# fegennari/3DWorld

Measured on AMD Instinct MI355X. Metric: heightmap Gcells/sec (noise+erosion), 16384^2 grid, higher is better.
Workload: dtype f32

## Files before the change

### 3dworld_amd/csrc/terra_driver.hpp

```cpp
#pragma once
#include "terra_common.hpp"
#include "terra_noise.hpp"
#include "terra_erosion.hpp"
#include "terra_landscape.hpp"
#include "terra_modmap.hpp"
#include "terra_treemap.hpp"
#include "terra_treeplace.hpp"
#include "terra_decidplace.hpp"
#include "terra_sceneryplace.hpp"
#include "terra_treeao.hpp"
#include "terra_treeedit.hpp"
#include "../../include/terra.h"
#include <vector>
#include <map>
#include <string>
#include <algorithm>
#include <cmath>
#include <stdexcept>
#include <string.h>
#include <stdio.h>
#include <stdlib.h>

namespace terra {

// ... 306 lines not shown
	for (int dy = -1; dy <= 1; ++dy) {
		for (int dx = -1; dx <= 1; ++dx) {
			if (dx == 0 && dy == 0) continue;
			float z0 = z_start;
			int stepx = dx, stepy = dy, vx = x, vy = y;
			for (unsigned s = 0; s < 8; ++s) {
				vx += stepx; vy += stepy;
				z0 += dz;
				stepx += dx; stepy += dy;
				if (ctx(vx + 36, vy + 36) > z0) {atten += (8 - s); break;}
			}
		}
	}
	float const ao_scale = (float)(1.0 - (double)((float)atten/(float)64));
	return (uint8_t)(255.0*(double)ao_scale);
}

TERRA_HD float rsq_approx(float x) {
#if defined(__HIP_DEVICE_COMPILE__)
	return __builtin_amdgcn_rsqf(x);
#else
	return (float)(1.0/sqrt((double)x));
#endif
}
TERRA_HD void tile_normal_v(float zc, float zr, float zd, float dxv, float dyv, float dxy, float nv[3]) {
	nv[0] = dyv*(zc - zr); nv[1] = dxv*(zc - zd); nv[2] = dxy;
	float const mag = sqrtf(nv[0]*nv[0] + nv[1]*nv[1] + nv[2]*nv[2]);
	if (!(mag < 1.0E-12f)) {nv[0] /= mag; nv[1] /= mag; nv[2] /= mag;}
}
TERRA_HD void tile_normal_zv(float const *z, unsigned zv, unsigned x, unsigned y, float dxv, float dyv, float dxy, float nv[3]) {
	unsigned const ix2 = y*zv + x;
	tile_normal_v(z[ix2], z[ix2 + 1], z[ix2 + zv], dxv, dyv, dxy, nv);
}

struct options_t {
	int gen_fused = 0;
	int ero_lead = 2;
	int ero_batch = 0;
	int ero_fuse = 3;
	int ero_sparse = -1;
	int ero_sparse_retraces = -1;
	int ero_live = 1;
	int ero_diag = 0;
	int ero_ck_steps = 0, ero_ck_max = -1;
	bool ero_near_set = false; int ero_near = 0;
	long long ero_mem_budget = -1;
	int simple_kernels = 0;
	int ao_bands = 1;
	int ao_whole = 1;
	int voxels_cols = 1;
	int graphs = 1;
	int sg_kc = 27, sg_kc_tiles = 27;
	int sg_rowgroup = 4;
	int tile_erosion_window = 0;
	int weights_simple = 0;
	int shadows_levels = 0;
	bool set(char const *key, char const *value) {
		if (!key || !value) return false;
		std::string const k(key), v(value);
		char *end = nullptr;
		long long const n = strtoll(value, &end, 10);
		bool const is_int = (end != value && *end == '\0');
		auto const flag = [&](int &dst) {if (!is_int || (n != 0 && n != 1)) return false; dst = (int)n; return true;};
		if (k == "gen.fused") {if (!is_int || n < 0 || n > 2) return false; gen_fused = (int)n; return true;}
		if (k == "ero.lead") {if (!is_int || n < 0 || n > 2) return false; ero_lead = (int)n; return true;}
		if (k == "ero.fuse") {if (!is_int || n < 0 || n > 7) return false; ero_fuse = (int)n; return true;}
		if (k == "ero.batch") {if (!is_int || n < 0 || n > (1 << 20)) return false; ero_batch = (int)n; return true;}
		if (k == "ero.sparse") {if (v == "auto") {ero_sparse = -1; return true;} return flag(ero_sparse);}
		if (k == "ero.sparse_retraces") {if (!is_int || n < -1 || n > (1 << 20)) return false; ero_sparse_retraces = (int)n; return true;}
		if (k == "ero.live") return flag(ero_live);
		if (k == "ero.diag") return flag(ero_diag);
		if (k == "ero.ck") {int a = 0, b = 0; if (v == "default") {ero_ck_steps = 0; ero_ck_max = -1; return true;} if (sscanf(value, "%d:%d", &a, &b) != 2 || a < 1 || b < 0 || b > (int)SPEC_CK_MAX) return false; ero_ck_steps = a; ero_ck_max = b; return true;}
		if (k == "ero.near") {if (v == "default") {ero_near_set = false; return true;} if (!is_int || n < -(1 << 20) || n > (1 << 20)) return false; ero_near_set = true; ero_near = (int)n; return true;}
		if (k == "ero.mem_budget") {if (!is_int || n < -1) return false; ero_mem_budget = n; return true;}
		if (k == "kernels.simple") return flag(simple_kernels);
		if (k == "voxels.cols") return flag(voxels_cols);
		if (k == "ao.bands") return flag(ao_bands);
		if (k == "ao.whole") return flag(ao_whole);
		if (k == "graphs") return flag(graphs);
		if (k == "sg.kc") {if (!is_int || (n != 20 && n != 27 && n != 45)) return false; sg_kc = (int)n; return true;}
		if (k == "sg.kc_tiles") {if (!is_int || (n != 27 && n != 45)) return false; sg_kc_tiles = (int)n; return true;}
		if (k == "sg.rowgroup") {if (!is_int || n < 1 || n > 1024) return false; sg_rowgroup = (int)n; return true;}
		if (k == "tile_erosion") {if (v == "lds") {tile_erosion_window = 0; return true;} if (v == "window") {tile_erosion_window = 1; return true;} return false;}
		if (k == "weights.simple") return flag(weights_simple);
		if (k == "shadows.levels") return flag(shadows_levels);
		return false;
	}
};

struct vox_noise_job_t {float l0, l1, l2, v0, v1, v2, o0, o1, o2, frx, fry, mag, freq, zscale; int32_t nn, normalize; uint32_t nx, nz, y0;};
TERRA_HD float voxel_noise_cell(size_t i, vox_noise_job_t const &J, bool perlin) {
	unsigned const z = (unsigned)(i % J.nz), x = (unsigned)((i / J.nz) % J.nx), y = (unsigned)(i / ((size_t)J.nz*J.nx)) + J.y0;
	float const px = ((float)x*J.v0 + J.l0) + J.o0, py = ((float)y*J.v1 + J.l1) + J.o1, pz = ((float)z*J.v2 + J.l2) + J.o2;
	float val = 0.0f, nmag = J.mag, nfreq = (float)(0.25*(double)J.freq);
	for (int n = 0; n < J.nn; ++n) {
		float const ax = nfreq*px + J.frx, ay = nfreq*py + J.fry, az = nfreq*pz + (J.frx - J.fry);
		val += nmag*(perlin ? perlin3(ax, ay, az) : simplex3(ax, ay, az));
		nmag *= 0.5f; nfreq *= 1.92f;
	}
	val += (float)z*J.zscale;
	if (J.normalize) {val = clip_pm1(val);}
	return val;
}

template<bool PERLIN> TERRA_HD nv2 voxel_noise_pair(unsigned x, unsigned y, unsigned z, vox_noise_job_t const &J, char const *tab) {
	float const px = ((float)x*J.v0 + J.l0) + J.o0, py = ((float)y*J.v1 + J.l1) + J.o1;
	nv2 const zf = {(float)z, (float)(z + 1)};
	nv2 const pz = (zf*J.v2 + J.l2) + J.o2;
	nv2 val = {0.0f, 0.0f};
	float nmag = J.mag, nfreq = (float)(0.25*(double)J.freq);
	float const frz = J.frx - J.fry;
	for (int n = 0; n < J.nn; ++n) {
		float const ax = nfreq*px + J.frx, ay = nfreq*py + J.fry;
		nv2 const az = nfreq*pz + frz;
		nv2 const v = PERLIN ? perlin3_lut_z2<true>(ax, ay, az, tab) : simplex3_lut<true>(nv2{ax, ax}, nv2{ay, ay}, az, tab);
		val += nmag*v;
		nmag *= 0.5f; nfreq *= 1.92f;
	}
	val += zf*J.zscale;
	if (J.normalize) {val = nv2{clip_pm1(val[0]), clip_pm1(val[1])};}
	return val;
}

template<class BE> struct terra_engine {
	BE be;
	options_t opt;
	terra_engine() {be.opt = &opt;}
	void set_option(char const *key, char const *value) {
		options_t o = opt;
		if (!o.set(key, value)) throw std::invalid_argument(std::string("terra_set_option: unknown key or bad value: ") + (key ? key : "(null)") + " = " + (value ? value : "(null)"));
		be.sync();
		opt = o;
		be.options_changed();
	}
	terra_config cfg{};
// ... 281 lines not shown
			sk.xconst[k] = ms2*sinTable[k][4] + sinTable[k][2] + x_mult*mx0;
			sk.yconst[k] = ms2*sinTable[k][3] + sinTable[k][1] + y_mult*my0;
			sk.xmdx[k] = x_mult*dx; sk.ymdy[k] = y_mult*dy;
		}
		return sk;
	}

	bool sine_plain_only(int shp, int kstart) const {
		if (shp != 0 || hp.crack_lo < hp.crack_hi || (hp.volcano_width > 0.0f && hp.volcano_height > 0.0f) || consts().custom_glaciate_exp != 0.0f) return false;
		double bound = 0.0;
		for (int k = kstart; k < F_TABLE_SIZE; ++k) {bound += std::fabs((double)(mesh_scale_z_inv*sinTable[k][0]));}
		return (double)min_std(hp.plat_bot, hp.crat_h) > bound*1.001 + 1e-3;
	}

	void gen_grid_dev(float x0, float y0, float dx, float dy, uint32_t nx, uint32_t ny, uint32_t flags, int min_start_sin, float *d_out, float *h_minmax = nullptr, uint32_t row0 = 0, uint32_t nrows = 0xFFFFFFFFu, float *d_minmax = nullptr) {
		require_scene();
		if (nx == 0 || ny == 0) throw std::invalid_argument("build_arrays: nx, ny must be > 0");
		if (nrows == 0xFFFFFFFFu) {if (row0 != 0) throw std::invalid_argument("gen_grid rows: row0 without a row count"); nrows = ny;}
		if (nrows == 0 || row0 >= ny || nrows > ny - row0) throw std::invalid_argument("gen_grid rows: [row0, row0 + nrows) must be a non-empty range inside the grid");
		grid_job_t job;
		job.mx0 = dx*x0; job.my0 = dy*y0; job.mdx = dx; job.mdy = dy; job.nx = nx; job.ny = nrows; job.row0 = row0; ny = nrows;
		job.nxp = round_up(nx, 128); job.nyp = round_up(ny, 128);
		bool const force_sine = (flags & TERRA_GEN_FORCE_SINE) != 0;
		job.mode = force_sine ? (int)MGEN_SINE : mode; job.shape = force_sine ? 0 : shape;
		job.kstart = imax(start_eval_sin, min_start_sin);
		job.glaciate = (flags & TERRA_GEN_GLACIATE) ? 1 : 0;
		job.use_sine_mag = (job.glaciate && hp.sine_mag > 0.0f) ? 1 : 0;
		job.sine_offset = hp.sine_bias*mesh_scale_z_inv;
		job.plain_only = (job.mode == MGEN_SINE && sine_plain_only(job.shape, job.kstart)) ? 1 : 0;
		job.fused = (((flags & (TERRA_GEN_FUSED | TERRA_GEN_FAST)) || opt.gen_fused) && fused_kernel_exists(job.mode, job.plain_only != 0)) ? (((flags & TERRA_GEN_FAST) || opt.gen_fused == 2) ? 2 : 1) : 0;
		job.fast_amax = sine_amp_max(job.kstart);
		noise_consts_t const nc = consts();
		sin_lut_t const L = lut();
		float *smx = scratch<float>(s_smx, job.nxp), *smy = scratch<float>(s_smy, job.nyp);
		uint32_t *d_mm = nullptr;
		bool const sine = (job.mode == MGEN_SINE);
		if (h_minmax || d_minmax || sine) {d_mm = scratch<uint32_t>(s_mm, 2); if (!sine) {be.fill32(d_mm, 0xFFFFFFFFu, 2);}}
		bool fused;
		bool const sm_on = job.use_sine_mag != 0;
		float const sm_scale = hp.sine_mag*mesh_scale_z_inv, sm_freq = mesh_scale*hp.sine_freq, dxi = DX_VAL_INV, dyi = DY_VAL_INV;
		if (sm_on && job.mode != MGEN_SINE) {
			float const mx0 = job.mx0, my0 = job.my0, mdx = dx, mdy = dy;
			uint32_t const nxp = job.nxp, nyp = job.nyp;
			be.launch((size_t)nxp + nyp, [=] TERRA_LAMBDA (size_t i) {
				if (i < nxp) {smx[i] = (i < nx) ? sm_scale*L.COSF(((float)(unsigned)i*mdx + mx0)*dxi*sm_freq) : 0.0f;}
				else {unsigned const y = (unsigned)(i - nxp); smy[y] = (y < ny) ? L.COSF(((float)(y + row0)*mdy + my0)*dyi*sm_freq) : 0.0f;}
			});
		}
		if (job.mode == MGEN_SINE) {
			float const *st = sinTable_dev();
			float const msx = mesh_scale*DX_VAL_INV, msy = mesh_scale*DY_VAL_INV, ms2 = (float)(0.5*(double)mesh_scale), mszi = mesh_scale_z_inv, jmx0 = job.mx0, jmy0 = job.my0, mdx = dx, mdy = dy;
			float *xt = scratch<float>(s_xt, (size_t)F_TABLE_SIZE*job.nxp), *yt = scratch<float>(s_yt, (size_t)F_TABLE_SIZE*job.nyp);
			uint32_t const nxp = job.nxp, nyp = job.nyp;
			size_t const ntab = (size_t)F_TABLE_SIZE*(nxp + nyp);
			uint32_t *const mmz = d_mm;
			be.launch(ntab + (sm_on ? (size_t)nxp + nyp : 0), [=] TERRA_LAMBDA (size_t i) {
				if (i == 0) {mmz[0] = 0xFFFFFFFFu; mmz[1] = 0xFFFFFFFFu;}
				if (i < (size_t)F_TABLE_SIZE*nxp) {
					unsigned const k = (unsigned)(i / nxp), x = (unsigned)(i % nxp);
					float const *stk = st + 5*k;
					float const x_mult = msx*stk[4], xconst = ms2*stk[4] + stk[2] + x_mult*jmx0, xmdx = x_mult*mdx;
					xt[i] = (x < nx) ? L.SINF(xmdx*(float)x + xconst) : 0.0f;
				}
				else if (i < ntab) {
					size_t const j = i - (size_t)F_TABLE_SIZE*nxp;
					unsigned const k = (unsigned)(j / nyp), y = (unsigned)(j % nyp);
					float const *stk = st + 5*k;
					float const y_mult = msy*stk[3], yscale = mszi*stk[0], yconst = ms2*stk[3] + stk[1] + y_mult*jmy0, ymdy = y_mult*mdy;
					yt[j] = (y < ny) ? yscale*L.SINF(ymdy*(float)(y + row0) + yconst) : 0.0f;
				}
				else {
					size_t const q = i - ntab;
					if (q < nxp) {smx[q] = (q < nx) ? sm_scale*L.COSF(((float)(unsigned)q*mdx + jmx0)*dxi*sm_freq) : 0.0f;}
					else {unsigned const y = (unsigned)(q - nxp); smy[y] = (y < ny) ? L.COSF(((float)(y + row0)*mdy + jmy0)*dyi*sm_freq) : 0.0f;}
				}
			});
			fused = be.sine_grid(job, nc, L, xt, yt, smx, smy, d_out, (h_minmax || d_minmax) ? d_mm : nullptr);
		}
		else {fused = be.noise_grid(job, nc, L, smx, smy, d_out, (h_minmax || d_minmax) ? d_mm : nullptr, d_noise_lut);}
		if ((h_minmax || d_minmax) && !fused) {be.minmax(d_out, (size_t)nx*ny, d_mm);}
		if (d_minmax) {uint32_t const *mm = d_mm; be.launch(1, [=] TERRA_LAMBDA (size_t) {d_minmax[0] = ord2f(mm[0]); d_minmax[1] = ord2f(~mm[1]);}, 64);}
		if (h_minmax) {
			uint32_t out[2];
			be.d2h(out, d_mm, sizeof(out));
			h_minmax[0] = ord2f(out[0]); h_minmax[1] = ord2f(~out[1]);
		}
	}

	float eval_mesh_sin_terms(float xv, float yv) const {
		require_scene();
		sin_lut_t const HL = host_lut();
		float zval = 0.0f;
		for (int k = start_eval_sin; k < F_TABLE_SIZE; ++k) {
			float const *stk = sinTable[k];
			zval += stk[0]*HL.SINF(stk[3]*yv + stk[1])*HL.SINF(stk[4]*xv + stk[2]);
		}
		return zval;
	}
	void eval_points_dev(float const *d_xy, uint32_t n, uint32_t kind, float xy_scale, int no_xyoff, int xoff2, int yoff2, float *d_out) {
		require_scene();
		if (n == 0) return;
		if (kind > 1) throw std::invalid_argument("eval_points: kind must be TERRA_POINTS_SCALED or TERRA_POINTS_EXACT");
		noise_consts_t const nc = consts();
		sin_lut_t const L = lut();
		float const *st = sinTable_dev();
		hmap_view_t const hv = hmap_view();
		bool const hm = using_hmap(), hm_detail = using_hmap_with_detail();
		int const md = mode, shp = shape, k0 = start_eval_sin;
		float const half_x = (float)(cfg.mesh_x >> 1), half_y = (float)(cfg.mesh_y >> 1), xss = cfg.scene_x, yss = cfg.scene_y, dxi = DX_VAL_INV, dyi = DY_VAL_INV, msc = mesh_scale, mszi = mesh_scale_z_inv;
		be.launch(n, [=] TERRA_LAMBDA (size_t i) {
			auto const scaled = [&](float xval, float yval, float xys) -> float {
				float const xv = xys*(xval - half_x), yv = xys*(yval - half_y);
				if (md != MGEN_SINE) {
					switch (md) {
					case MGEN_PERLIN:      return noise_zval<MGEN_PERLIN>(xv, yv, shp, nc);
					case MGEN_DWARP_GPU:   return noise_zval<MGEN_DWARP_GPU>(xv, yv, shp, nc);
					case MGEN_SIMPLEX_GPU: return noise_zval<MGEN_SIMPLEX_GPU>(xv, yv, shp, nc);
					default:               return noise_zval<MGEN_SIMPLEX>(xv, yv, shp, nc);
					}
				}
				float const ax = msc*xv, ay = msc*yv;
				float zval = 0.0f;
				for (int k = k0; k < F_TABLE_SIZE; ++k) {float const *stk = st + 5*k; zval += stk[0]*L.SINF(stk[3]*ay + stk[1])*L.SINF(stk[4]*ax + stk[2]);}
				return apply_noise_shape_final(zval*mszi, shp, nc.hp);
// ... 1832 lines not shown
```

### 3dworld_amd/csrc/terra_hip.hip

```cpp
#include "terra_kernels.hpp"
#include "terra_fused.hpp"
#include "terra_fz_api.hpp"
#include "terra_simple_paths.hpp"
#include "terra_xfer.hpp"
#include <stdlib.h>

#define TERRA_HIP_CHECK(expr) do {hipError_t const e_ = (expr); if (e_ != hipSuccess) {throw std::runtime_error(std::string(#expr) + ": " + hipGetErrorString(e_));}} while (0)

struct hip_backend_t : terra::simple_paths<hip_backend_t> {
	int device = -1;
	hipStream_t stream = nullptr, own_stream = nullptr;
	hipEvent_t ev0 = nullptr, ev1 = nullptr;
	terra::options_t const *opt = nullptr;
	bool simple_kernels = false;
	int num_cus = 256;
	float *tile_pad = nullptr; size_t tile_pad_bytes = 0;
	uint32_t *tile_order = nullptr; size_t tile_order_bytes = 0;
	float *vox_p = nullptr; size_t vox_p_bytes = 0;
	bool vox_cols = true;
	int sg_kc = 27;
	unsigned sg_rowgroup = 4;

	static int device_count() {int n = 0; if (hipGetDeviceCount(&n) != hipSuccess) return 0; return n;}
	void init(int dev) {
		device = dev;
		TERRA_HIP_CHECK(hipSetDevice(dev));
		TERRA_HIP_CHECK(hipStreamCreateWithFlags(&own_stream, hipStreamNonBlocking));
		stream = own_stream;
		TERRA_HIP_CHECK(hipEventCreate(&ev0)); TERRA_HIP_CHECK(hipEventCreate(&ev1));
		{int n = 0; if (hipDeviceGetAttribute(&n, hipDeviceAttributeMultiprocessorCount, dev) == hipSuccess && n > 0) {num_cus = n;} else {(void)hipGetLastError();}}
		options_changed();
		TERRA_HIP_CHECK(hipFuncSetAttribute((void const *)terra::k_tile_erosion, hipFuncAttributeMaxDynamicSharedMemorySize, 96*1024));
		TERRA_HIP_CHECK(hipFuncSetAttribute((void const *)terra::k_tile_shadows_level, hipFuncAttributeMaxDynamicSharedMemorySize, 96*1024));
		TERRA_HIP_CHECK(hipFuncSetAttribute((void const *)terra::k_tile_shadows_flow, hipFuncAttributeMaxDynamicSharedMemorySize, 96*1024));
		TERRA_HIP_CHECK(hipFuncSetAttribute((void const *)terra::k_tile_ao<true>, hipFuncAttributeMaxDynamicSharedMemorySize, 64*1024));
		TERRA_HIP_CHECK(hipFuncSetAttribute((void const *)terra::k_tile_ao<false>, hipFuncAttributeMaxDynamicSharedMemorySize, 64*1024));
		ao_tile_ok = hipFuncSetAttribute((void const *)terra::k_tile_ao_tile<true>, hipFuncAttributeMaxDynamicSharedMemorySize, (int)terra::AOT_LDS) == hipSuccess
			&& hipFuncSetAttribute((void const *)terra::k_tile_ao_tile<false>, hipFuncAttributeMaxDynamicSharedMemorySize, (int)terra::AOT_LDS) == hipSuccess;
		if (!ao_tile_ok) {(void)hipGetLastError();}
	}
	void options_changed() {
		if (!opt) return;
		simple_kernels = opt->simple_kernels != 0; sg_kc = opt->sg_kc; sg_rowgroup = (unsigned)opt->sg_rowgroup; vox_cols = opt->voxels_cols != 0;
		if (graphs_enabled != (opt->graphs != 0)) {for (graph_slot_t &g : graphs) {graph_drop(g);} graphs_enabled = opt->graphs != 0;}
	}
	~hip_backend_t() {
		if (pin) (void)hipHostFree(pin);
		if (h3_tab) (void)hipFree(h3_tab);
		if (tile_pad) (void)hipFree(tile_pad);
		if (tile_order) (void)hipFree(tile_order);
		if (tile_acc) (void)hipFree(tile_acc);
		if (tile_map) (void)hipFree(tile_map);
		if (vox_p) (void)hipFree(vox_p);
		if (ev0) (void)hipEventDestroy(ev0);
		if (ev1) (void)hipEventDestroy(ev1);
		for (graph_slot_t &g : graphs) {graph_drop(g);}
		if (relay_ev) (void)hipEventDestroy(relay_ev);
		if (side_stream) (void)hipStreamDestroy(side_stream);
		if (own_stream) (void)hipStreamDestroy(own_stream);
	}
	size_t mem_free() {use(); size_t f = 0, t = 0; if (hipMemGetInfo(&f, &t) != hipSuccess) {(void)hipGetLastError(); return ~(size_t)0 >> 1;} return f;}
	void release_scratch() {
		for (void **p : {(void **)&tile_pad, (void **)&tile_order, (void **)&tile_acc, (void **)&tile_map, (void **)&vox_p}) {if (*p) {(void)hipFree(*p); *p = nullptr;}}
		tile_pad_bytes = tile_order_bytes = tile_acc_bytes = vox_p_bytes = 0; tile_map_count = 0;
	}
	void use() {TERRA_HIP_CHECK(hipSetDevice(device));}
	void set_stream(void *s) {sync(); pin_off = 0; stream = s ? (hipStream_t)s : own_stream;}
	void sync() {use(); TERRA_HIP_CHECK(hipStreamSynchronize(stream));}
	void *alloc(size_t bytes) {use(); void *p = nullptr; TERRA_HIP_CHECK(hipMalloc(&p, bytes ? bytes : 1)); return p;}
	void free(void *p) {use(); (void)hipFree(p);}
	void fill8(void *p, uint8_t v, size_t count) {use(); if (count) TERRA_HIP_CHECK(hipMemsetAsync(p, v, count, stream));}
	void fill32(void *p, uint32_t v, size_t count) {use(); if (count) TERRA_HIP_CHECK(hipMemsetD32Async((hipDeviceptr_t)p, (int)v, count, stream));}
	void h2d(void *d, void const *h, size_t bytes) {
		use();
		if (bytes >= BIG_XFER) {xfer.submit(device, stream, const_cast<void *>(h), d, bytes, true, [this](hipEvent_t e) {return record_via_side(e);}); xfer.wait_all(); return;}
		TERRA_HIP_CHECK(hipMemcpyAsync(d, h, bytes, hipMemcpyHostToDevice, stream)); TERRA_HIP_CHECK(hipStreamSynchronize(stream));
	}
	uint8_t *pin = nullptr; size_t pin_bytes = 0, pin_off = 0; bool pin_failed = false;
	void h2d_async(void *d, void const *h, size_t bytes) {
		if (bytes == 0) return;
		use();
		if (!pin && !pin_failed) {pin_bytes = (size_t)8 << 20; if (hipHostMalloc((void **)&pin, pin_bytes, hipHostMallocDefault) != hipSuccess) {pin = nullptr; pin_bytes = 0; pin_failed = true; (void)hipGetLastError();}}
		size_t const need = (bytes + 255) & ~(size_t)255;
		if (!pin || need > pin_bytes/2) {h2d(d, h, bytes); return;}
		if (pin_off + need > pin_bytes) {TERRA_HIP_CHECK(hipStreamSynchronize(stream)); pin_off = 0;}
		memcpy(pin + pin_off, h, bytes);
		TERRA_HIP_CHECK(hipMemcpyAsync(d, pin + pin_off, bytes, hipMemcpyHostToDevice, stream));
		pin_off += need;
	}
	void d2h(void *h, void const *d, size_t bytes) {
		use();
		if (bytes >= BIG_XFER) {download_async(d, h, bytes); download_wait(); return;}
		TERRA_HIP_CHECK(hipMemcpyAsync(h, d, bytes, hipMemcpyDeviceToHost, stream)); TERRA_HIP_CHECK(hipStreamSynchronize(stream));
	}
	static constexpr size_t BIG_XFER = (size_t)16 << 20;
	terra::xfer_engine_t xfer;
// ... 120 lines not shown

	template<class F> void launch_waves_lean(size_t n, F f) {
		if (n == 0) return;
		use();
		if (n > 0x7FFFFFFFull) throw std::invalid_argument("launch_waves: grid too large");
		hipLaunchKernelGGL(terra::k_waves_lean<F>, dim3((unsigned)n), dim3(64), 0, stream, f);
		TERRA_HIP_CHECK(hipGetLastError());
	}

	template<class F> void launch_waves_nolds(size_t n, F f) {
		if (n == 0) return;
		use();
		if (n > 0x7FFFFFFFull) throw std::invalid_argument("launch_waves: grid too large");
		hipLaunchKernelGGL(terra::k_waves_nolds<F>, dim3((unsigned)n), dim3(64), 0, stream, f);
		TERRA_HIP_CHECK(hipGetLastError());
	}

	void *h3_tab = nullptr; size_t h3_tab_bytes = 0;
	static float h3_scale(float amax) {int e = 0; if (amax > 0.0f && amax < 3.0e38f) {(void)frexpf(amax, &e);} return ldexpf(1.0f, 14 - e);}
	template<int KIND> bool sine_grid_h3(terra::sgf_job_t J, float amax_x, float amax_y, float const *vox_tab = nullptr, uint32_t vnx = 0, uint32_t vny = 0) {
		int const nk = (J.kstart < J.kend) ? J.kend - J.kstart : 0;
		uint32_t const nchunks = (uint32_t)((3*nk + 15)/16);
		if ((uint64_t)std::max(J.nxp, J.nyp)*32u*(nchunks + 1) >= 0xFFFFFFFFull) return false;
		size_t const bx = (size_t)nchunks*J.nxp*32u, by = (size_t)nchunks*J.nyp*32u;
		if (bx + by + 64 > h3_tab_bytes) {if (h3_tab) {sync(); (void)hipFree(h3_tab);} TERRA_HIP_CHECK(hipMalloc(&h3_tab, bx + by + 64)); h3_tab_bytes = bx + by + 64;}
		float const sx = h3_scale(amax_x), sy = h3_scale(amax_y);
		J.xh = h3_tab; J.yh = (char *)h3_tab + bx; J.nchunks = nchunks; J.unscale = 1.0f/(sx*sy);
		if (nchunks && vox_tab) {
			hipLaunchKernelGGL((terra::k_split_voxel_table<false, terra::VOX_SINES>), dim3((J.nxp + 255)/256), dim3(256), 0, stream, vox_tab, vnx, vny, J.nx, J.nxp, sx, (terra::sgh_u4 *)J.xh);
			hipLaunchKernelGGL((terra::k_split_voxel_table<true, terra::VOX_SINES>),  dim3((J.nyp + 255)/256), dim3(256), 0, stream, vox_tab, vnx, vny, J.nx, J.nyp, sy, (terra::sgh_u4 *)J.yh);
		}
		else if (nchunks) {
			hipLaunchKernelGGL(terra::k_split_table<false>, dim3((unsigned)(((size_t)nchunks*J.nxp + 255)/256)), dim3(256), 0, stream, J.xt, J.nxp, J.kstart, J.kend, nchunks, sx, (terra::sgh_u4 *)J.xh);
			hipLaunchKernelGGL(terra::k_split_table<true>,  dim3((unsigned)(((size_t)nchunks*J.nyp + 255)/256)), dim3(256), 0, stream, J.yt, J.nyp, J.kstart, J.kend, nchunks, sy, (terra::sgh_u4 *)J.yh);
		}
		if (KIND == terra::SGF_VOXELS && J.nx <= 64 && (J.nyp % 256u) == 0) {J.narrow = 1; J.ntx = 1; J.nty = J.nyp/256u;}
		unsigned const nb = J.ntx*J.nty, grid = ((nb + 7)/8)*8;
		hipLaunchKernelGGL(terra::k_sine_grid_h3<KIND>, dim3(grid), dim3(256), 0, stream, J);
		TERRA_HIP_CHECK(hipGetLastError());
		return true;
	}
	bool sine_grid(terra::grid_job_t const &job, terra::noise_consts_t const &nc, terra::sin_lut_t const &L, float const *xt, float const *yt, float const *smx, float const *smy, float *out, uint32_t *mm) {
		if (simple_kernels) {sine_grid_simple(job, nc, L, xt, yt, smx, smy, out); return false;}
		use();
		unsigned const ntx = job.nxp/terra::SG_BX, nty = (job.ny + terra::SG_BY - 1)/terra::SG_BY;
		unsigned const nb = ntx*nty, grid = ((nb + 7)/8)*8;
		if (job.fused) {
			terra::sgf_job_t J; memset(&J, 0, sizeof(J));
			J.xt = xt; J.yt = yt; J.smx = smx; J.smy = smy; J.out = out; J.mm = mm; J.nx = job.nx; J.ny = job.ny; J.nxp = job.nxp; J.nyp = job.nyp; J.ntx = ntx; J.nty = nty; J.rowgroup = sg_rowgroup;
			J.kstart = job.kstart; J.kend = terra::F_TABLE_SIZE; J.glaciate = (job.glaciate && nc.glaciate) ? 1 : 0; J.sine_mag = (job.glaciate && job.use_sine_mag) ? 1 : 0;
			J.zmax_est = nc.zmax_est; J.zmax_est2 = nc.zmax_est2; J.zmax_est2_inv = nc.zmax_est2_inv; J.sine_offset = job.sine_offset;
			if (job.fused == 2 && sine_grid_h3<terra::SGF_GRID>(J, 1.0f, job.fast_amax)) return true;
			hipLaunchKernelGGL(terra::k_sine_grid_mx<terra::SGF_GRID>, dim3(std::min(grid, (unsigned)(2*num_cus + 7)/8*8)), dim3(256), 0, stream, J);
			TERRA_HIP_CHECK(hipGetLastError());
			return true;
		}
		terra::sg_tiles_t const tl{nullptr, nullptr, 0, sg_rowgroup, 0, 0, 0, 0xFFFFFFFFu, 0, 0xFFFFFFFFu, 0};
		if (job.plain_only) {
			auto const go = [&](auto kern) {hipLaunchKernelGGL(kern, dim3(grid), dim3(terra::SG_THREADS), 0, stream, job, nc, L, xt, yt, smx, smy, out, ntx, nty, mm, tl);};
			if (sg_kc == 27) go(terra::k_sine_grid<false, false, 27>); else if (sg_kc == 20) go(terra::k_sine_grid<false, false, 20>); else go(terra::k_sine_grid<false, false, 45>);
		}
		else                {hipLaunchKernelGGL((terra::k_sine_grid<false, true>),  dim3(grid), dim3(terra::SG_THREADS), 0, stream, job, nc, L, xt, yt, smx, smy, out, ntx, nty, mm, tl);}
		TERRA_HIP_CHECK(hipGetLastError());
		return true;
	}
	bool noise_grid(terra::grid_job_t const &job, terra::noise_consts_t const &nc, terra::sin_lut_t const &L, float const *smx, float const *smy, float *out, uint32_t *mm, uint32_t const *nlut) {
		if (simple_kernels) {noise_grid_simple(job, nc, L, smx, smy, out); return false;}
		use();
		if (job.fused) {TERRA_HIP_CHECK((hipError_t)terra_fz_noise_grid(job.mode, &job, &nc, &L, smx, smy, out, mm, nlut, (void *)stream)); return true;}
		dim3 const grid((job.nx + 127)/128, (job.ny + terra::NG_ROWS - 1)/terra::NG_ROWS), block(256);
		terra::noise_oct_t const oc = terra::make_noise_oct(nc);
		switch (job.mode) {
		case terra::MGEN_PERLIN:      hipLaunchKernelGGL(terra::k_noise_grid<terra::MGEN_PERLIN>,      grid, block, 0, stream, job, nc, L, smx, smy, out, mm, nlut, oc); break;
		case terra::MGEN_DWARP_GPU:   hipLaunchKernelGGL(terra::k_noise_grid<terra::MGEN_DWARP_GPU>,   grid, block, 0, stream, job, nc, L, smx, smy, out, mm, nlut, oc); break;
		case terra::MGEN_SIMPLEX_GPU: hipLaunchKernelGGL(terra::k_noise_grid<terra::MGEN_SIMPLEX_GPU>, grid, block, 0, stream, job, nc, L, smx, smy, out, mm, nlut, oc); break;
		default:                      hipLaunchKernelGGL(terra::k_noise_grid<terra::MGEN_SIMPLEX>,     grid, block, 0, stream, job, nc, L, smx, smy, out, mm, nlut, oc); break;
		}
		TERRA_HIP_CHECK(hipGetLastError());
		return true;
	}
	int32_t *tile_map = nullptr; size_t tile_map_count = 0;
	bool tile_band_ok(uint32_t n, uint32_t nux, uint32_t nuy, uint32_t twx, bool unique_tiles, bool plain_only, int md) const {
		return !simple_kernels && md == terra::MGEN_SINE && unique_tiles && plain_only && (uint64_t)n*2 >= (uint64_t)nux*nuy && ((nux*twx) & 3u) == 0 && (!opt || opt->sg_kc_tiles == 27) && (!opt || opt->ao_bands != 0);
	}
	void tile_grid(uint32_t n, terra::tile_ref_pod_t const *refs, uint32_t nux, uint32_t nuy, float const *xt, float const *yt, uint32_t nxpv, uint32_t nypv, float const *d_sm, float const *d_m0,
		int md, int shp, int kstart, bool use_sm, float so, terra::noise_consts_t const &nc, terra::sin_lut_t const &L, float dxv, float dyv, float *zvals, bool plain_only, uint32_t tw, bool unique_tiles, bool glaciate = true, uint32_t const *nlut = nullptr, int fused = 0, float fast_amax = 0.0f,
		terra::tile_band_t const *band = nullptr)
	{
		if (!simple_kernels && md != terra::MGEN_SINE) {
			use();
			terra::grid_job_t job;
			job.mx0 = 0; job.my0 = 0; job.mdx = dxv; job.mdy = dyv; job.nx = job.ny = tw; job.nxp = nxpv; job.nyp = nypv;
			job.mode = md; job.shape = shp; job.kstart = kstart; job.glaciate = glaciate ? 1 : 0; job.use_sine_mag = use_sm ? 1 : 0; job.sine_offset = so; job.plain_only = 0;
			if (fused) {TERRA_HIP_CHECK((hipError_t)terra_fz_noise_tiles(refs, n, nux, d_sm, d_m0, &job, &nc, &L, zvals, tw, nlut, (void *)stream)); return;}
			terra::noise_oct_t const oc = terra::make_noise_oct(nc);
			size_t const threads = (size_t)n*tw*((tw + 1)/2);
			dim3 const grid((unsigned)((threads + 255)/256)), block(256);
			switch (md) {
			case terra::MGEN_PERLIN:      hipLaunchKernelGGL(terra::k_noise_tiles<terra::MGEN_PERLIN>,      grid, block, 0, stream, refs, n, nux, d_sm, d_m0, job, nc, L, zvals, tw, nlut, oc); break;
			case terra::MGEN_DWARP_GPU:   hipLaunchKernelGGL(terra::k_noise_tiles<terra::MGEN_DWARP_GPU>,   grid, block, 0, stream, refs, n, nux, d_sm, d_m0, job, nc, L, zvals, tw, nlut, oc); break;
			case terra::MGEN_SIMPLEX_GPU: hipLaunchKernelGGL(terra::k_noise_tiles<terra::MGEN_SIMPLEX_GPU>, grid, block, 0, stream, refs, n, nux, d_sm, d_m0, job, nc, L, zvals, tw, nlut, oc); break;
			default:                      hipLaunchKernelGGL(terra::k_noise_tiles<terra::MGEN_SIMPLEX>,     grid, block, 0, stream, refs, n, nux, d_sm, d_m0, job, nc, L, zvals, tw, nlut, oc); break;
			}
			TERRA_HIP_CHECK(hipGetLastError());
			return;
		}
// ... 346 lines not shown
```

### 3dworld_amd/csrc/terra_kernels.hpp

```cpp
#pragma once
#include "terra_driver.hpp"
#include "terra_noise_kernels.hpp"

namespace terra {

typedef float    st_f4 __attribute__((ext_vector_type(4)));
typedef uint32_t st_u4 __attribute__((ext_vector_type(4)));

template<class F> __global__ void k_generic(size_t n, F f) {
	size_t const i = (size_t)blockIdx.x*blockDim.x + threadIdx.x;
	if (i < n) {f(i);}
}

template<class F> __global__ __launch_bounds__(64) void k_waves(F f, unsigned first) {
	__builtin_amdgcn_s_setprio(3);
	__shared__ __attribute__((aligned(16))) float win[EW*EW];
	__shared__ uint8_t dirty[EW*EW];
	__shared__ wave_shared_t sh;
	wave_scratch_t const ws{win, dirty, &sh};
	f((size_t)blockIdx.x + first, ws);
}

template<class F> __global__ __launch_bounds__(64) void k_waves_nolds(F f) {f((size_t)blockIdx.x);}

// ... 239 lines not shown
				float z = acc[i][half*2 + (j >> 1)][j & 1];
				if (!GENERAL || (plain && !(z > pp_limit))) {
					if (job.glaciate) {
						if (nc.glaciate) {float const relh = (z + nc.zmax_est)*nc.zmax_est2_inv; z = (GENERAL ? glaciate_exp_fn(relh, nc.custom_glaciate_exp) : relh*relh*relh)*nc.zmax_est2 - nc.zmax_est;}
						if (job.use_sine_mag) {z += smxv[half*4 + j]*smyv[i] + job.sine_offset;}
					}
				}
				else if (GENERAL && x + j < job.nx) {
					if (TILES) {
						unsigned const tw = tiles.tw, ux = (x + j)/tw, uy = y/tw;
						grid_job_t jt = job; jt.mx0 = tiles.m0[ux]; jt.my0 = tiles.m0[tiles.nux + uy];
						z = finish_cell(z, jt, nc, L, smx + ux*tw, smy + uy*tw, (x + j) - ux*tw, y - uy*tw);
					}
					else {z = finish_cell(z, job, nc, L, smx, smy, x + j, y);}
				}
				else {z = 0.0f;}
				v[j] = z;
				if (x + j < job.nx) {fmn = fminf(fmn, z); fmx = fmaxf(fmx, z);}
			}
			if (TILES) {
				unsigned const tw = tiles.tw;
				unsigned uy = t_uy[i >> 2], cy = t_cy[i >> 2] + (unsigned)(i & 3);
				if (cy >= tw) {cy -= tw; ++uy;}
				if ((tw & 1u) == 0) {
#pragma unroll
					for (int j = 0; j < 4; j += 2) {
						if (x + j >= job.nx) continue;
						unsigned ux = t_ux[half], cx = t_cx[half] + (unsigned)j;
						if (cx >= tw) {cx -= tw; ++ux;}
						int const t = tiles.tile_map[uy*tiles.nux + ux];
						if (t >= 0) {*(float2 *)(out + (size_t)t*tw*tw + cy*tw + cx) = make_float2(v[j], v[j + 1]);}
					}
					continue;
				}
#pragma unroll
				for (int j = 0; j < 4; ++j) {
					if (x + j >= job.nx) continue;
					unsigned ux = t_ux[half], cx = t_cx[half] + (unsigned)j;
					if (cx >= tw) {cx -= tw; ++ux;}
					int const t = tiles.tile_map[uy*tiles.nux + ux];
					if (t >= 0) {out[(size_t)t*tw*tw + cy*tw + cx] = v[j];}
				}
				continue;
			}
			float *o = out + (size_t)y*job.nx + x;
			if (vec_ok) {*(float4 *)o = make_float4(v[0], v[1], v[2], v[3]);}
			else {
#pragma unroll
				for (int j = 0; j < 4; ++j) {if (x + j < job.nx) o[j] = v[j];}
			}
		}
	}
	if (mm) {
		if (fmn <= fmx) {mm_lo = f2ord(fmn); mm_hi = ~f2ord(fmx);}
		wave_minmax_publish(mm_lo, mm_hi, mm);
	}
}

__global__ __launch_bounds__(256) void k_tile_land_cells(float const *__restrict__ zvals, uint32_t cells, float water_thresh, uint32_t *__restrict__ land) {
	float const *z = zvals + (size_t)blockIdx.x*cells;
	uint32_t cnt = 0;
	for (uint32_t i = threadIdx.x; i < cells; i += 256) {cnt += !(z[i] < water_thresh) ? 1u : 0u;}
#pragma unroll
	for (int off = 32; off > 0; off >>= 1) {cnt += __shfl_down(cnt, off, 64);}
	if ((threadIdx.x & 63) == 0 && cnt) {atomicAdd(&land[blockIdx.x], cnt);}
}
__global__ __launch_bounds__(256) void k_tile_order_by_land(uint32_t const *__restrict__ land, uint32_t n, uint32_t *__restrict__ order) {
	__shared__ uint32_t s_land[256];
	uint32_t const i = blockIdx.x*256 + threadIdx.x;
	uint32_t const mine = (i < n) ? land[i] : 0u;
	uint32_t pos = 0;
	for (uint32_t j0 = 0; j0 < n; j0 += 256) {
		__syncthreads();
		s_land[threadIdx.x] = (j0 + threadIdx.x < n) ? land[j0 + threadIdx.x] : 0u;
		__syncthreads();
		uint32_t const cnt = (n - j0 < 256u) ? n - j0 : 256u;
		for (uint32_t e = 0; e < cnt; ++e) {uint32_t const l = s_land[e]; pos += (l > mine || (l == mine && j0 + e < i)) ? 1u : 0u;}
	}
	if (i < n) {order[pos] = i;}
}
__global__ __launch_bounds__(64) void k_tile_erosion(float *__restrict__ zvals, erosion_consts_t ec, uint32_t iters, uint32_t const *__restrict__ order, uint32_t const *__restrict__ land) {
	extern __shared__ __attribute__((aligned(16))) float te_pad[];
	int const NX = ec.NX, NY = ec.NY, xs = ec.xsize, ys = ec.ysize;
	uint32_t const tile = order ? order[blockIdx.x] : blockIdx.x;
	float *z = zvals + (size_t)tile*xs*ys;
	if (land && land[tile] == 0) {
		for (int i = threadIdx.x; i < xs*ys; i += 64) {z[i] = max_std(ec.min_zval, z[i]);}
		return;
	}
	for (int i = threadIdx.x; i < NX*NY; i += 64) {
		int const X = i % NX, Z = i / NX;
		te_pad[i] = z[(size_t)imax(imin(Z - EROSION_PAD, ys-1), 0)*xs + imax(imin(X - EROSION_PAD, xs-1), 0)];
	}
	__syncthreads();
	{
		wave_lds_mem_t m; m.pad = te_pad; m.NX = NX; m.NY = NY;
		for (uint32_t it = 0; it < iters; ++it) {simulate_droplet((int)it, m, ec);}
	}
	__syncthreads();
	for (int i = threadIdx.x; i < xs*ys; i += 64) {
		int const x = i % xs, y = i / xs;
		z[i] = max_std(ec.min_zval, te_pad[(y + EROSION_PAD)*NX + (x + EROSION_PAD)]);
	}
}

__device__ __forceinline__ uint32_t wave_min_u32(uint32_t v) {
// ... 1497 lines not shown
```

### 3dworld_amd/terra.py

```python
import ctypes as C
import os
import numpy as np

HERE = os.path.dirname(os.path.abspath(__file__))

GEN_GLACIATE, GEN_FORCE_SINE, GEN_NO_WAIT, GEN_CACHE_VALUES, GEN_FUSED, GEN_FAST = 1, 2, 4, 8, 16, 32
ERODE_SERIAL, ERODE_MINZ_IS_MIN, ERODE_SERIAL_WAVE = 1, 2, 4
MGEN_SINE, MGEN_SIMPLEX, MGEN_PERLIN, MGEN_SIMPLEX_GPU, MGEN_DWARP_GPU = range(5)


class TerraError(RuntimeError):
    def __init__(self, code, msg):
        super().__init__(f"terra error {code}: {msg}")
        self.code = code


class Config(C.Structure):
    _fields_ = [("mesh_x", C.c_int32), ("mesh_y", C.c_int32), ("scene_x", C.c_float), ("scene_y", C.c_float), ("scene_z", C.c_float),
                ("mesh_height", C.c_float), ("mesh_scale", C.c_float), ("mesh_seed", C.c_int32), ("mesh_freq_filter", C.c_int32),
                ("mesh_gen_mode", C.c_int32), ("mesh_gen_shape", C.c_int32), ("glaciate", C.c_int32), ("custom_glaciate_exp", C.c_float),
                ("hmap", C.c_float * 14), ("erode_amount", C.c_float), ("water_h_off", C.c_float), ("water_h_off_rel", C.c_float),
                ("relh_adj_tex", C.c_float), ("ocean_wave_height", C.c_float),
                ("start_mag", C.c_float), ("start_freq", C.c_float), ("mag_mult", C.c_float), ("freq_mult", C.c_float)]

# ... 325 lines not shown
        raise TerraError(-1, lib.terra_last_error().decode())
    out = np.empty((h.value, w.value, 2) if nc.value == 2 else (h.value, w.value), np.uint8)
    if lib.terra_heightmap_read_png(*args, out.ctypes.data, out.nbytes) < 0:
        raise TerraError(-1, lib.terra_last_error().decode())
    return out


class DeviceBuffer:

    def __init__(self, terra, nbytes):
        self.t, self.nbytes = terra, nbytes
        p = _vp()
        terra._ck(terra.lib.terra_malloc(terra.ctx, C.byref(p), nbytes))
        self.ptr = p.value

    def upload(self, arr):
        arr = np.ascontiguousarray(arr)
        assert arr.nbytes <= self.nbytes
        self.t._ck(self.t.lib.terra_memcpy_h2d(self.t.ctx, self.ptr, arr.ctypes.data, arr.nbytes))
        return self

    def download(self, dtype, shape):
        out = np.empty(shape, dtype)
        assert out.nbytes <= self.nbytes
        self.t._ck(self.t.lib.terra_memcpy_d2h(self.t.ctx, out.ctypes.data, self.ptr, out.nbytes))
        return out

    def free(self):
        if self.ptr:
            self.t.lib.terra_free(self.t.ctx, self.ptr)
            self.ptr = None


class PinnedArray:

    def __init__(self, lib, shape, dtype=np.float32):
        self.lib = lib
        n = int(np.prod(shape)) * np.dtype(dtype).itemsize
        lib.terra_host_alloc.restype = _vp
        self.ptr = lib.terra_host_alloc(max(n, 1))
        if not self.ptr:
            raise TerraError(-1, lib.terra_last_error().decode())
        self.array = np.frombuffer((C.c_uint8 * n).from_address(self.ptr), dtype=dtype).reshape(shape)

    def free(self):
        if self.ptr:
            self.array = None
            self.lib.terra_host_free(self.ptr)
            self.ptr = None


ENV_OPTIONS = {
    "TERRA_GEN_FUSED": ("gen.fused", "0"), "TERRA_SIMPLE_KERNELS": ("kernels.simple", "0"), "TERRA_GRAPHS": ("graphs", "1"),
    "TERRA_SG_KC": ("sg.kc", "27"), "TERRA_SG_KC_TILES": ("sg.kc_tiles", "27"), "TERRA_SG_ROWGROUP": ("sg.rowgroup", "4"), "TERRA_TILE_EROSION": ("tile_erosion", "lds"),
    "TERRA_WEIGHTS_SIMPLE": ("weights.simple", "0"), "TERRA_VOXELS_COLS": ("voxels.cols", "1"), "TERRA_AO_BANDS": ("ao.bands", "1"), "TERRA_AO_WHOLE": ("ao.whole", "1"), "TERRA_SHADOWS_LEVELS": ("shadows.levels", "0"),
    "TERRA_ERO_SPARSE": ("ero.sparse", "auto"), "TERRA_ERO_SPARSE_RETRACES": ("ero.sparse_retraces", "-1"), "TERRA_ERO_LEAD": ("ero.lead", "2"), "TERRA_ERO_BATCH": ("ero.batch", "0"), "TERRA_ERO_FUSE": ("ero.fuse", "3"),
    "TERRA_ERO_LIVE": ("ero.live", "1"), "TERRA_ERO_DIAG": ("ero.diag", "0"), "TERRA_ERO_CK": ("ero.ck", "default"), "TERRA_ERO_NEAR": ("ero.near", "default"),
    "TERRA_ERO_MEM_BUDGET": ("ero.mem_budget", "-1"),
}


class Terra:

    def __init__(self, device=0, lib_path=None, env_options=True):
        self.lib = load_library(lib_path)
        ctx = _vp()
        rc = self.lib.terra_create(C.byref(ctx), device)
        if rc != 0:
            raise TerraError(rc, self.lib.terra_last_error().decode())
        self.ctx = ctx
        self._env_applied = {}
        if env_options:
            self.apply_env_options()

    def set_option(self, key, value):
        self._ck(self.lib.terra_set_option(self.ctx, str(key).encode(), str(value).encode()))

    def apply_env_options(self):
        for var, (key, default) in ENV_OPTIONS.items():
            val = os.environ.get(var, default)
            if self._env_applied.get(key, default) != val:
                self.set_option(key, val)
                self._env_applied[key] = val

    def close(self):
        if getattr(self, "ctx", None):
            self.lib.terra_destroy(self.ctx)
            self.ctx = None

    def __del__(self):
        try:
            self.close()
        except Exception:
            pass

    def _ck(self, rc):
        if rc < 0:
            raise TerraError(rc, self.lib.terra_last_error().decode())
        return rc

    def init_scene(self, cfg):
        self._ck(self.lib.terra_init_scene(self.ctx, C.byref(cfg)))
        return self.state()

    def state(self):
        s = State()
        self._ck(self.lib.terra_get_state(self.ctx, C.byref(s)))
# ... 766 lines not shown
```

Measured before the change: 322.2.

## Add opt-in register-blocked sine grid kernel and skip unused table rows

Adds k_sine_grid_sy, a sine-sum grid kernel in which each lane accumulates a 4-column by 16-row block in registers. It uses packed f32 inline asm, buffer loads for the x tables and scalar-register y rows, with a triple-buffered load pipeline. The kernel only runs when the new sg.sy option is enabled, which defaults to 0. Separately, the table-building launch now fills only the rows from kstart onward instead of all F_TABLE_SIZE rows, which changes work on the default path. The new kernel adds inline asm and an address-space cast, which are correctness and portability risks once it is enabled.

```diff
diff --git a/3dworld_amd/csrc/terra_driver.hpp b/3dworld_amd/csrc/terra_driver.hpp
--- a/3dworld_amd/csrc/terra_driver.hpp
+++ b/3dworld_amd/csrc/terra_driver.hpp
@@ -382,6 +382,7 @@
 	int graphs = 1;
 	int sg_kc = 27, sg_kc_tiles = 27;
 	int sg_rowgroup = 4;
+	int sg_sy = 0;
 	int tile_erosion_window = 0;
 	int weights_simple = 0;
 	int shadows_levels = 0;
@@ -411,6 +412,7 @@
 		if (k == "sg.kc") {if (!is_int || (n != 20 && n != 27 && n != 45)) return false; sg_kc = (int)n; return true;}
 		if (k == "sg.kc_tiles") {if (!is_int || (n != 27 && n != 45)) return false; sg_kc_tiles = (int)n; return true;}
 		if (k == "sg.rowgroup") {if (!is_int || n < 1 || n > 1024) return false; sg_rowgroup = (int)n; return true;}
+		if (k == "sg.sy") return flag(sg_sy);
 		if (k == "tile_erosion") {if (v == "lds") {tile_erosion_window = 0; return true;} if (v == "window") {tile_erosion_window = 1; return true;} return false;}
 		if (k == "weights.simple") return flag(weights_simple);
 		if (k == "shadows.levels") return flag(shadows_levels);
@@ -798,24 +800,25 @@
 			float const msx = mesh_scale*DX_VAL_INV, msy = mesh_scale*DY_VAL_INV, ms2 = (float)(0.5*(double)mesh_scale), mszi = mesh_scale_z_inv, jmx0 = job.mx0, jmy0 = job.my0, mdx = dx, mdy = dy;
 			float *xt = scratch<float>(s_xt, (size_t)F_TABLE_SIZE*job.nxp), *yt = scratch<float>(s_yt, (size_t)F_TABLE_SIZE*job.nyp);
 			uint32_t const nxp = job.nxp, nyp = job.nyp;
-			size_t const ntab = (size_t)F_TABLE_SIZE*(nxp + nyp);
+			unsigned const k0 = (unsigned)imin(imax(job.kstart, 0), F_TABLE_SIZE), nkb = (unsigned)F_TABLE_SIZE - k0;
+			size_t const nxtab = (size_t)nkb*nxp, ntab = nxtab + (size_t)nkb*nyp;
 			uint32_t *const mmz = d_mm;
-			be.launch(ntab + (sm_on ? (size_t)nxp + nyp : 0), [=] TERRA_LAMBDA (size_t i) {
+			be.launch(std::max<size_t>(ntab + (sm_on ? (size_t)nxp + nyp : 0), 1), [=] TERRA_LAMBDA (size_t i) {
 				if (i == 0) {mmz[0] = 0xFFFFFFFFu; mmz[1] = 0xFFFFFFFFu;}
-				if (i < (size_t)F_TABLE_SIZE*nxp) {
-					unsigned const k = (unsigned)(i / nxp), x = (unsigned)(i % nxp);
+				if (i < nxtab) {
+					unsigned const k = k0 + (unsigned)(i / nxp), x = (unsigned)(i % nxp);
 					float const *stk = st + 5*k;
 					float const x_mult = msx*stk[4], xconst = ms2*stk[4] + stk[2] + x_mult*jmx0, xmdx = x_mult*mdx;
-					xt[i] = (x < nx) ? L.SINF(xmdx*(float)x + xconst) : 0.0f;
+					xt[(size_t)k*nxp + x] = (x < nx) ? L.SINF(xmdx*(float)x + xconst) : 0.0f;
 				}
 				else if (i < ntab) {
-					size_t const j = i - (size_t)F_TABLE_SIZE*nxp;
-					unsigned const k = (unsigned)(j / nyp), y = (unsigned)(j % nyp);
+					size_t const j = i - nxtab;
+					unsigned const k = k0 + (unsigned)(j / nyp), y = (unsigned)(j % nyp);
 					float const *stk = st + 5*k;
 					float const y_mult = msy*stk[3], yscale = mszi*stk[0], yconst = ms2*stk[3] + stk[1] + y_mult*jmy0, ymdy = y_mult*mdy;
-					yt[j] = (y < ny) ? yscale*L.SINF(ymdy*(float)(y + row0) + yconst) : 0.0f;
-				}
-				else {
+					yt[(size_t)k*nyp + y] = (y < ny) ? yscale*L.SINF(ymdy*(float)(y + row0) + yconst) : 0.0f;
+				}
+				else if (sm_on) {
 					size_t const q = i - ntab;
 					if (q < nxp) {smx[q] = (q < nx) ? sm_scale*L.COSF(((float)(unsigned)q*mdx + jmx0)*dxi*sm_freq) : 0.0f;}
 					else {unsigned const y = (unsigned)(q - nxp); smy[y] = (y < ny) ? L.COSF(((float)(y + row0)*mdy + jmy0)*dyi*sm_freq) : 0.0f;}
diff --git a/3dworld_amd/csrc/terra_hip.hip b/3dworld_amd/csrc/terra_hip.hip
--- a/3dworld_amd/csrc/terra_hip.hip
+++ b/3dworld_amd/csrc/terra_hip.hip
@@ -20,6 +20,7 @@
 	bool vox_cols = true;
 	int sg_kc = 27;
 	unsigned sg_rowgroup = 4;
+	bool sg_sy = false;
 
 	static int device_count() {int n = 0; if (hipGetDeviceCount(&n) != hipSuccess) return 0; return n;}
 	void init(int dev) {
@@ -41,7 +42,7 @@
 	}
 	void options_changed() {
 		if (!opt) return;
-		simple_kernels = opt->simple_kernels != 0; sg_kc = opt->sg_kc; sg_rowgroup = (unsigned)opt->sg_rowgroup; vox_cols = opt->voxels_cols != 0;
+		simple_kernels = opt->simple_kernels != 0; sg_kc = opt->sg_kc; sg_rowgroup = (unsigned)opt->sg_rowgroup; sg_sy = opt->sg_sy != 0; vox_cols = opt->voxels_cols != 0;
 		if (graphs_enabled != (opt->graphs != 0)) {for (graph_slot_t &g : graphs) {graph_drop(g);} graphs_enabled = opt->graphs != 0;}
 	}
 	~hip_backend_t() {
@@ -268,6 +269,12 @@
 			J.zmax_est = nc.zmax_est; J.zmax_est2 = nc.zmax_est2; J.zmax_est2_inv = nc.zmax_est2_inv; J.sine_offset = job.sine_offset;
 			if (job.fused == 2 && sine_grid_h3<terra::SGF_GRID>(J, 1.0f, job.fast_amax)) return true;
 			hipLaunchKernelGGL(terra::k_sine_grid_mx<terra::SGF_GRID>, dim3(std::min(grid, (unsigned)(2*num_cus + 7)/8*8)), dim3(256), 0, stream, J);
+			TERRA_HIP_CHECK(hipGetLastError());
+			return true;
+		}
+		if (job.plain_only && (job.nx & 3u) == 0 && sg_sy && (uint64_t)terra::F_TABLE_SIZE*job.nxp*4u < 0xFFFFFFFFull) {
+			unsigned const sntx = (job.nx + terra::SY_BX - 1)/terra::SY_BX, snty = (job.ny + terra::SY_BY - 1)/terra::SY_BY;
+			hipLaunchKernelGGL(terra::k_sine_grid_sy, dim3((sntx*snty + 7)/8*8), dim3(256), 0, stream, job, nc, xt, yt, smx, smy, out, sntx, snty, 2u*sg_rowgroup, mm);
 			TERRA_HIP_CHECK(hipGetLastError());
 			return true;
 		}
diff --git a/3dworld_amd/csrc/terra_kernels.hpp b/3dworld_amd/csrc/terra_kernels.hpp
--- a/3dworld_amd/csrc/terra_kernels.hpp
+++ b/3dworld_amd/csrc/terra_kernels.hpp
@@ -315,6 +315,106 @@
 		}
 	}
 	if (mm) {
+		if (fmn <= fmx) {mm_lo = f2ord(fmn); mm_hi = ~f2ord(fmx);}
+		wave_minmax_publish(mm_lo, mm_hi, mm);
+	}
+}
+
+constexpr int SY_BX = 256, SY_BY = 64, SY_ROWS = 16;
+typedef float sy_f4  __attribute__((ext_vector_type(4)));
+typedef float sy_f16 __attribute__((ext_vector_type(16)));
+typedef __attribute__((address_space(4))) sy_f16 const sy_cf16;
+__device__ __forceinline__ sy_f16 sy_load_rows(float const *p) {return *(sy_cf16 *)(uintptr_t)p;}
+__device__ __forceinline__ void sy_mul_add_4x4(sg_v2f &a00, sg_v2f &a01, sg_v2f &a10, sg_v2f &a11, sg_v2f &a20, sg_v2f &a21, sg_v2f &a30, sg_v2f &a31, sg_v2f x0, sg_v2f x1, sg_v2f ya, sg_v2f yb) {
+	sg_v2f t0, t1;
+#define TERRA_SY_2X2(A0, A1, X, Y) \
+	"v_pk_mul_f32 %8, " X ", " Y " op_sel:[0,0] op_sel_hi:[1,0]\n\t" \
+	"v_pk_mul_f32 %9, " X ", " Y " op_sel:[0,1] op_sel_hi:[1,1]\n\t" \
+	"v_pk_add_f32 " A0 ", " A0 ", %8\n\t" \
+	"v_pk_add_f32 " A1 ", " A1 ", %9\n\t"
+	asm(TERRA_SY_2X2("%0", "%2", "%10", "%12") TERRA_SY_2X2("%1", "%3", "%11", "%12") TERRA_SY_2X2("%4", "%6", "%10", "%13") TERRA_SY_2X2("%5", "%7", "%11", "%13")
+	    : "+v"(a00), "+v"(a01), "+v"(a10), "+v"(a11), "+v"(a20), "+v"(a21), "+v"(a30), "+v"(a31), "=&v"(t0), "=&v"(t1)
+	    : "v"(x0), "v"(x1), "s"(ya), "s"(yb));
+#undef TERRA_SY_2X2
+}
+__device__ __forceinline__ void sy_accumulate_rows4(sg_v2f (&acc)[SY_ROWS][2], sy_f4 const &x, sy_f16 const &y, int q) {
+	sy_mul_add_4x4(acc[4*q][0], acc[4*q][1], acc[4*q + 1][0], acc[4*q + 1][1], acc[4*q + 2][0], acc[4*q + 2][1], acc[4*q + 3][0], acc[4*q + 3][1],
+		sg_v2f{x.x, x.y}, sg_v2f{x.z, x.w}, sg_v2f{y[4*q], y[4*q + 1]}, sg_v2f{y[4*q + 2], y[4*q + 3]});
+}
+
+__global__ __launch_bounds__(256) void k_sine_grid_sy(grid_job_t job, noise_consts_t nc, float const *__restrict__ xt, float const *__restrict__ yt, float const *__restrict__ smx,
+	float const *__restrict__ smy, float *__restrict__ out, unsigned ntx, unsigned nty, unsigned rowgroup, uint32_t *__restrict__ mm)
+{
+	unsigned bxi, byi;
+	if (!sg_tile_of_block(blockIdx.x, ntx, nty, rowgroup, bxi, byi)) return;
+	unsigned const wave = __builtin_amdgcn_readfirstlane(threadIdx.x >> 6), lane = threadIdx.x & 63u;
+	unsigned const row0 = byi*SY_BY + wave*SY_ROWS, x = bxi*SY_BX + lane*4u;
+	if (row0 >= job.ny) return;
+	bool const col_ok = x < job.nx;
+	unsigned const xoff = ((x + 4u <= job.nxp) ? x : job.nxp - 4u)*4u;
+	sg_v2f acc[SY_ROWS][2];
+#pragma unroll
+	for (int r = 0; r < SY_ROWS; ++r) {acc[r][0] = sg_v2f{0.0f, 0.0f}; acc[r][1] = sg_v2f{0.0f, 0.0f};}
+	int kn = (job.kstart < F_TABLE_SIZE - 1) ? ((job.kstart > 0) ? job.kstart : 0) : F_TABLE_SIZE - 1, n = F_TABLE_SIZE - job.kstart;
+	__amdgpu_buffer_rsrc_t const rx = __builtin_amdgcn_make_buffer_rsrc(const_cast<float *>(xt), 0, 0xFFFFFFFFu, 0x00020000);
+	uint32_t const xstep = job.nxp*4u;
+	uint32_t sxn = (uint32_t)kn*xstep;
+	float const *pyn = yt + (size_t)kn*job.nyp + row0;
+	auto const next_row = [&]() {if (kn < F_TABLE_SIZE - 1) {++kn; sxn += xstep; pyn += job.nyp;}};
+	auto const load_x = [&]() -> sy_f4 {return __builtin_bit_cast(sy_f4, __builtin_amdgcn_raw_buffer_load_b128(rx, xoff, sxn, 0));};
+	sy_f4 XA, XB, XC; sy_f16 YA, YB, YC;
+	XA = load_x(); YA = sy_load_rows(pyn); next_row();
+	XB = load_x(); YB = sy_load_rows(pyn); next_row();
+#define TERRA_SY_TERM(XS, YS, XT, YT) \
+	XT = load_x(); __builtin_amdgcn_sched_barrier(0); \
+	sy_accumulate_rows4(acc, XS, YS, 0); __builtin_amdgcn_sched_barrier(0); \
+	YT = sy_load_rows(pyn); next_row(); __builtin_amdgcn_sched_barrier(0); \
+	sy_accumulate_rows4(acc, XS, YS, 1); sy_accumulate_rows4(acc, XS, YS, 2); sy_accumulate_rows4(acc, XS, YS, 3); __builtin_amdgcn_sched_barrier(0);
+	for (; n >= 3; n -= 3) {
+		TERRA_SY_TERM(XA, YA, XC, YC)
+		TERRA_SY_TERM(XB, YB, XA, YA)
+		TERRA_SY_TERM(XC, YC, XB, YB)
+	}
+#undef TERRA_SY_TERM
+	if (n >= 1) {
+#pragma unroll
+		for (int q = 0; q < 4; ++q) {sy_accumulate_rows4(acc, XA, YA, q);}
+	}
+	if (n >= 2) {
+#pragma unroll
+		for (int q = 0; q < 4; ++q) {sy_accumulate_rows4(acc, XB, YB, q);}
+	}
+	typedef sg_v2f v2f;
+	bool const gl = job.glaciate && nc.glaciate, sm = job.glaciate && job.use_sine_mag;
+	v2f const zme = {nc.zmax_est, nc.zmax_est}, inv = {nc.zmax_est2_inv, nc.zmax_est2_inv}, z2 = {nc.zmax_est2, nc.zmax_est2}, off = {job.sine_offset, job.sine_offset};
+	float fmn = INFINITY, fmx = -INFINITY;
+	if (col_ok) {
+		sy_f4 sx = {0.0f, 0.0f, 0.0f, 0.0f}; sy_f16 sy = {};
+		if (sm) {sx = *(sy_f4 const *)(smx + x); sy = sy_load_rows(smy + row0);}
+		v2f const s01 = {sx.x, sx.y}, s23 = {sx.z, sx.w};
+		char *po = (char *)(out + (size_t)row0*job.nx);
+		size_t const ostep = (size_t)job.nx*4u;
+		unsigned const rows = (job.ny - row0 < (unsigned)SY_ROWS) ? job.ny - row0 : (unsigned)SY_ROWS;
+#pragma unroll
+		for (int r = 0; r < SY_ROWS; ++r) {
+			if ((unsigned)r >= rows) continue;
+			v2f z01 = acc[r][0], z23 = acc[r][1];
+			if (gl) {
+				v2f const r01 = (z01 + zme)*inv, r23 = (z23 + zme)*inv;
+				z01 = ((r01*r01)*r01)*z2 - zme; z23 = ((r23*r23)*r23)*z2 - zme;
+			}
+			if (sm) {
+				v2f const syi = {sy[r], sy[r]};
+				z01 = z01 + (s01*syi + off); z23 = z23 + (s23*syi + off);
+			}
+			fmn = sg_min3(sg_min3(fmn, z01.x, z01.y), z23.x, z23.y);
+			fmx = sg_max3(sg_max3(fmx, z01.x, z01.y), z23.x, z23.y);
+			*(sy_f4 *)(po + x*4u) = sy_f4{z01.x, z01.y, z23.x, z23.y};
+			po += ostep;
+		}
+	}
+	if (mm) {
+		uint32_t mm_lo = 0xFFFFFFFFu, mm_hi = 0xFFFFFFFFu;
 		if (fmn <= fmx) {mm_lo = f2ord(fmn); mm_hi = ~f2ord(fmx);}
 		wave_minmax_publish(mm_lo, mm_hi, mm);
 	}
diff --git a/3dworld_amd/terra.py b/3dworld_amd/terra.py
--- a/3dworld_amd/terra.py
+++ b/3dworld_amd/terra.py
@@ -401,7 +401,7 @@
 
 ENV_OPTIONS = {
     "TERRA_GEN_FUSED": ("gen.fused", "0"), "TERRA_SIMPLE_KERNELS": ("kernels.simple", "0"), "TERRA_GRAPHS": ("graphs", "1"),
-    "TERRA_SG_KC": ("sg.kc", "27"), "TERRA_SG_KC_TILES": ("sg.kc_tiles", "27"), "TERRA_SG_ROWGROUP": ("sg.rowgroup", "4"), "TERRA_TILE_EROSION": ("tile_erosion", "lds"),
+    "TERRA_SG_KC": ("sg.kc", "27"), "TERRA_SG_KC_TILES": ("sg.kc_tiles", "27"), "TERRA_SG_ROWGROUP": ("sg.rowgroup", "4"), "TERRA_SG_SY": ("sg.sy", "0"), "TERRA_TILE_EROSION": ("tile_erosion", "lds"),
     "TERRA_WEIGHTS_SIMPLE": ("weights.simple", "0"), "TERRA_VOXELS_COLS": ("voxels.cols", "1"), "TERRA_AO_BANDS": ("ao.bands", "1"), "TERRA_AO_WHOLE": ("ao.whole", "1"), "TERRA_SHADOWS_LEVELS": ("shadows.levels", "0"),
     "TERRA_ERO_SPARSE": ("ero.sparse", "auto"), "TERRA_ERO_SPARSE_RETRACES": ("ero.sparse_retraces", "-1"), "TERRA_ERO_LEAD": ("ero.lead", "2"), "TERRA_ERO_BATCH": ("ero.batch", "0"), "TERRA_ERO_FUSE": ("ero.fuse", "3"),
     "TERRA_ERO_LIVE": ("ero.live", "1"), "TERRA_ERO_DIAG": ("ero.diag", "0"), "TERRA_ERO_CK": ("ero.ck", "default"), "TERRA_ERO_NEAR": ("ero.near", "default"),
```

Result: slower. 313.1 (-2.8%).
